# RTCartist/Neuromorphic-Spatiotemporal-Optical-Flow

Measured on AMD Instinct MI355X. Metric: 1080p frame-pairs/sec (Farneback, HIP), higher is better.
Workload: dtype f32

## Files before the change

include/nsof.h:

```cpp
#ifndef NSOF_H
#define NSOF_H

#include <stddef.h>
#include <stdint.h>

#ifdef __cplusplus
extern "C" {
#endif

#define NSOF_ABI_VERSION 3

typedef enum nsof_status {
    NSOF_OK = 0,
    NSOF_EINVAL = -1,
    NSOF_ESHAPE = -2,
    NSOF_EDEVICE = -3,
    NSOF_ENOMEM = -4,
    NSOF_EUNSUPPORTED = -5
} nsof_status;

typedef struct nsof_ctx nsof_ctx;

int nsof_create(int device, nsof_ctx** out);
void nsof_destroy(nsof_ctx* ctx);
// ... 131 lines not shown
                                       const int32_t* d_rects, int max_rects, float* d_flows, double pyr_scale, int levels,
                                       int winsize, int iterations, int poly_n, double poly_sigma, int flags,
                                       int gate_frame, long long* n_calls, long long* n_pixels);
int nsof_farneback_f32_roi_sequence_dev(nsof_ctx* ctx, int n_frames, const float* d_frames, ptrdiff_t row_stride,
                                        ptrdiff_t frame_stride, int width, int height, const int32_t* d_counts,
                                        const int32_t* d_rects, int max_rects, float* d_flows, double pyr_scale, int levels,
                                        int winsize, int iterations, int poly_n, double poly_sigma, int flags,
                                        int gate_frame, long long* n_calls, long long* n_pixels);
void* nsof_host_alloc(size_t bytes);
void nsof_host_free(void* p);

int nsof_farneback_effective_levels(int width, int height, double pyr_scale, int levels);
int nsof_farneback_level_size(int width, int height, double pyr_scale, int level,
                              int* level_width, int* level_height, int* blur_ksize, double* blur_sigma);

int nsof_stage_pyr_level_px(nsof_ctx* ctx, int pixel_type, int n_img, const void* d_src, ptrdiff_t row_stride,
                            ptrdiff_t img_stride, int width, int height, double pyr_scale, int level, float* d_out);
int nsof_stage_pyr_level(nsof_ctx* ctx, int n_img, const uint8_t* d_src, ptrdiff_t row_stride,
                         ptrdiff_t img_stride, int width, int height, double pyr_scale, int level, float* d_out);
int nsof_stage_pyr_level_f32(nsof_ctx* ctx, int n_img, const float* d_src, ptrdiff_t row_stride,
                             ptrdiff_t img_stride, int width, int height, double pyr_scale, int level, float* d_out);
int nsof_stage_polyexp(nsof_ctx* ctx, int n_img, const float* d_img, int width, int height,
                       int poly_n, double poly_sigma, float* d_R);
int nsof_stage_recip(nsof_ctx* ctx, long long n, const double* d_x, double* d_out, double* d_ieee);
int nsof_stage_update_matrices(nsof_ctx* ctx, int n_pairs, const float* d_R, const float* d_flow,
                               int width, int height, float* d_M);
int nsof_stage_blur_solve(nsof_ctx* ctx, int n_pairs, const float* d_M, int width, int height,
                          int winsize, float* d_flow);
int nsof_stage_gauss_blur_solve(nsof_ctx* ctx, int n_pairs, const float* d_M, int width, int height,
                                int winsize, float* d_flow);
int nsof_stage_iterate(nsof_ctx* ctx, int n_pairs, const float* d_R, const float* d_flow_in, int width, int height,
                       int winsize, float* d_flow_out);
int nsof_stage_iterate_upsample(nsof_ctx* ctx, int n_pairs, const float* d_R, const float* d_coarse_flow,
                                int src_w, int src_h, int width, int height, int winsize, double pyr_scale,
                                float* d_flow_out);
int nsof_stage_flow_upsample(nsof_ctx* ctx, int n_pairs, const float* d_src, int src_w, int src_h,
                             float* d_dst, int dst_w, int dst_h, double pyr_scale);

typedef enum nsof_kernel_id {
    NSOF_K_PREP = 0,
    NSOF_K_POLYEXP = 1,
    NSOF_K_UPSAMPLE = 2,
    NSOF_K_UPDMAT = 3,
    NSOF_K_BLUR = 4,
    NSOF_K_ACCUM = 5,
    NSOF_K_ITERATE = 6,
// ... 118 lines not shown
```

neuromorphic-spatiotemporal-optical-flow_amd/csrc/farneback_kernels.hip:

```cpp
#include <cstdlib>

#include <type_traits>

#include "nsof_internal.h"

#ifdef NSOF_PYR_FMA
#define NSOF_MADD(a, b, c) fmaf((a), (b), (c))
#define NSOF_PYR_NAME(n) n##_fma
#else
#define NSOF_MADD(a, b, c) ((a) * (b) + (c))
#define NSOF_PYR_NAME(n) n
#endif

namespace {

__device__ __forceinline__ int reflect101(int p, int len)
{
    if ((unsigned)p < (unsigned)len) return p;
    if (len == 1) return 0;
    do {
        if (p < 0) p = -p;
        else p = 2 * len - 2 - p;
    } while ((unsigned)p >= (unsigned)len);
    return p;
}

__device__ __forceinline__ void lin_coord_x(int d, double scale, int slen, int& s, float& a)
{
    float f = (float)((d + 0.5) * scale - 0.5);
    s = floor_f(f);
    a = f - s;
    if (s < 0) { s = 0; a = 0.f; }
    if (s >= slen - 1) { s = slen - 1; a = 0.f; }
}
__device__ __forceinline__ void lin_coord_y(int d, double scale, int& s, float& a)
{
    float f = (float)((d + 0.5) * scale - 0.5);
    s = floor_f(f);
    a = f - s;
}


template <typename T>
__device__ __forceinline__ float px(const T* p) { return (float)*p; }
template <typename T>
__device__ __forceinline__ const T* srow(const T* img, ptrdiff_t r, ptrdiff_t stride)
{
    return reinterpret_cast<const T*>(reinterpret_cast<const char*>(img) + r * stride);
}
template <typename T>
constexpr bool kU8 = std::is_same<T, uint8_t>::value;
template <typename T>
constexpr bool kInt = std::is_integral<T>::value;
template <typename T>
constexpr int kPPD = kInt<T> ? 4 / (int)sizeof(T) : 1;
template <typename T>
// ... 913 lines not shown
#pragma unroll
            for (int p = 0; p < 4; p++) st[wave][4 * lane + (p ^ ((lane >> 1) & 3))] = make_float4(o0[p], o1[p], o2[p], o3[p]);
        }
        {
            const int yo2 = y + wave;
            float4* q4 = reinterpret_cast<float4*>(Rb) + (unsigned)yo2 * (unsigned)W + (unsigned)x0;
#pragma unroll
            for (int k = 0; k < 4; k++) {
                const int px = 64 * k + lane;
                const float4 v = st[wave][(px & ~3) | ((px & 3) ^ ((px >> 3) & 3))];
                if (px < G::SW && yo2 < ye && x0 + px < W) nsof_store_stream4(reinterpret_cast<float*>(q4 + px), v.x, v.y, v.z, v.w);
            }
        }
    }
}

struct PolyFrame {
    const uint8_t* src0;
    const uint8_t* src1;
    long long row_stride, img_stride;
    int nsplit;
    float k0, k1;
};
template <int N, bool HET, bool FRAME = false, typename SRC = uint8_t>
__global__ __launch_bounds__(512, N <= 7 ? 8 : 1) void k_polyexp_rs(const float* __restrict__ img, float* __restrict__ R, int W, int H,
                                                     int seg_rows, nsof_poly_taps tp,
                                                     const nsof_het_item* __restrict__ items, PolyFrame fr = PolyFrame{})
{
    using G = PolyGeom<N>;
    size_t img_off, r_off;
    const uint8_t* sb = nullptr;
    long long srs = 0;
    if constexpr (HET) {
        const nsof_het_item& it = items[blockIdx.z >> 1];
        const size_t which = blockIdx.z & 1;
        W = it.wk;
        H = it.hk;
        if (blockIdx.x * G::SW >= W || blockIdx.y * seg_rows >= H) return;
        img_off = it.offI + which * (size_t)W * H;
        r_off = it.offR + which * 5 * (size_t)W * H;
        if constexpr (FRAME) {
            sb = it.src[which];
            srs = it.src_stride[which];
        }
    } else {
        img_off = (size_t)blockIdx.z * W * H;
        r_off = (size_t)blockIdx.z * 5 * W * H;
        if constexpr (FRAME) {
            const int z = blockIdx.z;
            sb = z < fr.nsplit ? fr.src0 + (ptrdiff_t)z * fr.img_stride : fr.src1 + (ptrdiff_t)(z - fr.nsplit) * fr.img_stride;
            srs = fr.row_stride;
// ... 19 lines not shown
        using RawPx = std::conditional_t<std::is_signed<SRC>::value, int, unsigned>;
        struct Raw3 {
            RawPx l, c, r;
        };
        auto fetch3 = [&](int srow) {
            const SRC* rp = reinterpret_cast<const SRC*>(sb + (ptrdiff_t)srow * srs);
            return Raw3{rp[xl], rp[xc], rp[xr]};
        };
        auto hval = [&](const Raw3& q) { return NSOF_MADD((float)q.l + (float)q.r, fr.k1, (float)q.c * fr.k0); };
        int rc_cur = 0;
        float hm = 0.f, h0 = 0.f, hp = 0.f, icur = 0.f;
        auto below = [&](int row) { return reflect101(clampi(row, 0, H - 1) + 1, H); };
        auto advance = [&](int row, const Raw3& under) {
            const int rc = clampi(row, 0, H - 1);
            if (rc != rc_cur) {
                hm = h0;
                h0 = hp;
                hp = hval(under);
                icur = NSOF_MADD(hm + hp, fr.k1, h0 * fr.k0);
                rc_cur = rc;
            }
            return icur;
        };
        float win[2 * N + 1];
        float pre[4];
        Raw3 praw[4];
        if constexpr (FRAME) {
            rc_cur = clampi(ys - N, 0, H - 1);
            hm = hval(fetch3(reflect101(rc_cur - 1, H)));
            h0 = hval(fetch3(rc_cur));
            hp = hval(fetch3(reflect101(rc_cur + 1, H)));
            icur = NSOF_MADD(hm + hp, fr.k1, h0 * fr.k0);
            win[0] = icur;
#pragma unroll
            for (int j = 1; j <= 2 * N; j++) win[j] = advance(ys - N + j, fetch3(below(ys - N + j)));
#pragma unroll
            for (int q = 0; q < 4; q++) pre[q] = advance(ys + 1 + N + q, fetch3(below(ys + 1 + N + q)));
        } else {
#pragma unroll
            for (int j = 0; j <= 2 * N; j++) win[j] = ld(ys - N + j);
#pragma unroll
            for (int q = 0; q < 4; q++) pre[q] = ld(ys + 1 + N + q);
        }
        for (int t = 0; t <= nsteps; t++) {
            if (t < nsteps) {
                const int y = ys + 4 * t, buf = t & 1;
// ... 6 lines not shown
#pragma unroll
                for (int q = 0; q < 4; q++) {
                    float t0 = win[N] * tp.g[0], t1 = 0.f, t2 = 0.f;
#pragma unroll
                    for (int k = 1; k <= N; k++) {
                        const float a = win[N - k], b = win[N + k];
                        float p = a + b;
                        t0 = t0 + tp.g[k] * p;
                        t2 = t2 + tp.xxg[k] * p;
                        p = b - a;
                        t1 = t1 + tp.xg[k] * p;
                    }
                    sr[buf][0][q][tid] = t0;
                    sr[buf][1][q][tid] = t1;
                    sr[buf][2][q][tid] = t2;
#pragma unroll
                    for (int j = 0; j < 2 * N; j++) win[j] = win[j + 1];
                    win[2 * N] = pre[q];
                }
#pragma unroll
                for (int q = 0; q < 4; q++) {
                    if constexpr (FRAME) pre[q] = advance(y + 5 + N + q, praw[q]);
                    else pre[q] = nxt[q];
                }
            }
            __syncthreads();
        }
        return;
    }

    char* Rb = reinterpret_cast<char*>(R + r_off);
    for (int t = 0; t <= nsteps; t++) {
        if (t >= 1) {
            const int y = ys + 4 * (t - 1), buf = (t - 1) & 1;
            const int yo = y + wave;
            const int xo = x0 + 4 * lane;
            if (4 * lane < G::SW && yo < ye && xo < W) {
                const unsigned opix = (unsigned)yo * (unsigned)W + (unsigned)xo;
                auto load_row = [&](int a, float (&v)[4 * G::NV]) {
                    const float4* p4 = reinterpret_cast<const float4*>(&sr[buf][a][wave][4 * lane]);
#pragma unroll
                    for (int i = 0; i < G::NV; i++) {
                        const float4 f = p4[i];
                        v[4 * i] = f.x; v[4 * i + 1] = f.y; v[4 * i + 2] = f.z; v[4 * i + 3] = f.w;
                    }
                };
// ... 380 lines not shown
            rb = r1;
        }
        if (live) {
            float2 o[NPL];
#pragma unroll
            for (int i = 0; i < NPL; i++) {
                const float2 t0 = hA[i], t1 = same ? hA[i] : hB[i];
                o[i].x = NSOF_MADD(t0.x, b0, t1.x * b1) * mul;
                o[i].y = NSOF_MADD(t0.y, b0, t1.y * b1) * mul;
            }
            float2* drow = D + (size_t)dy * dw + dx0;
            if (dx0 + 1 < dw && (dw & 1) == 0) {
                nsof_store_stream4(reinterpret_cast<float*>(drow), o[0].x, o[0].y, o[1].x, o[1].y);
            } else {
                drow[0] = o[0];
                if (dx0 + 1 < dw) drow[1] = o[1];
            }
        }
    }
}

template <int N, typename SRC = uint8_t>
void launch_polyexp_n(nsof_ctx* ctx, int n_img, const float* img, int W, int H, const nsof_poly_taps& taps, float* R,
                      const PolyFrame* fr = nullptr)
{
    using G = PolyGeom<N>;
    const int strips = (W + G::SW - 1) / G::SW;
    int segs = 1;
    while (segs < 64 && (long long)strips * n_img * segs < 2048 && (H / (segs * 2)) >= 64) segs *= 2;
    while (segs < 128 && (long long)strips * n_img * segs < 256 && (H / (segs * 2)) >= 16) segs *= 2;
    int seg_rows = ((H + segs - 1) / segs + 3) / 4 * 4;
    segs = (H + seg_rows - 1) / seg_rows;
    dim3 grid(strips, segs, n_img);
    if (fr)
        hipLaunchKernelGGL((k_polyexp_rs<N, false, true, SRC>), grid, dim3(512), 0, ctx->stream, img, R, W, H, seg_rows, taps, nullptr, *fr);
    else if (ctx->opt_polyexp_f32)
        hipLaunchKernelGGL((k_polyexp<N>), grid, dim3(256), 0, ctx->stream, img, R, W, H, seg_rows, taps, nullptr);
    else
        hipLaunchKernelGGL((k_polyexp_rs<N, false>), grid, dim3(512), 0, ctx->stream, img, R, W, H, seg_rows, taps, nullptr);
}

template <int N, typename SRC = uint8_t>
void launch_polyexp_het_n(nsof_ctx* ctx, int n_img, const nsof_het_item* items, const float* img, int W, int H,
                          const nsof_poly_taps& taps, float* R, const PolyFrame* fr = nullptr)
{
    using G = PolyGeom<N>;
    const int strips = (W + G::SW - 1) / G::SW;
    int segs = 1;
    while (segs < 64 && (long long)strips * n_img * segs < 2048 && (H / (segs * 2)) >= 64) segs *= 2;
    int seg_rows = ((H + segs - 1) / segs + 3) / 4 * 4;
    segs = (H + seg_rows - 1) / seg_rows;
    dim3 grid(strips, segs, n_img);
    if (fr) hipLaunchKernelGGL((k_polyexp_rs<N, true, true, SRC>), grid, dim3(512), 0, ctx->stream, img, R, W, H, seg_rows, taps, items, *fr);
    else hipLaunchKernelGGL((k_polyexp_rs<N, true>), grid, dim3(512), 0, ctx->stream, img, R, W, H, seg_rows, taps, items);
}

}

namespace {
template <typename T>
int prep_decim3_impl(nsof_ctx* ctx, int n_img, const T* src, ptrdiff_t row_stride, ptrdiff_t img_stride, int W, int H,
                     const nsof_blur_taps* taps, float* const* out)
{
    const int CWL = (W & 15) == 0 && kU8<T> ? 16 : 8;
    const int AL = kU8<T> ? CWL : 8;
    const bool ok = (W & 7) == 0 && (H & 7) == 0 && W >= 64 && H > 19 && (row_stride % AL) == 0 && (img_stride % AL) == 0 &&
                    (reinterpret_cast<uintptr_t>(src) % AL) == 0 && taps[0].ksize == 3 && taps[1].ksize == 9 &&
                    taps[2].ksize == 19 && n_img <= 65535;
    if (!ok) return NSOF_EUNSUPPORTED;
    nsof_prof_scope ps(ctx, NSOF_K_PREP);
    Decim3 d;
    for (int k = 0; k < 3; k++) {
        d.t[k] = taps[k];
        d.out[k] = out[k];
    }
    int src_rows = 96;
// ... 137 lines not shown
{
    switch (src_type) {
        case NSOF_SRC_U8: return prep_decim3_impl(ctx, n_img, static_cast<const uint8_t*>(src), row_stride, img_stride, W, H, taps, out);
        case NSOF_SRC_U16: return prep_decim3_impl(ctx, n_img, static_cast<const uint16_t*>(src), row_stride, img_stride, W, H, taps, out);
        case NSOF_SRC_S16: return prep_decim3_impl(ctx, n_img, static_cast<const int16_t*>(src), row_stride, img_stride, W, H, taps, out);
        default: return NSOF_EUNSUPPORTED;
    }
}

int NSOF_PYR_NAME(nsof_launch_prep)(nsof_ctx* ctx, int n_img, const void* src, ptrdiff_t row_stride, ptrdiff_t img_stride, int W,
                                    int H, int wk, int hk, const nsof_blur_taps& taps, float* out, int src_type)
{
    switch (src_type) {
        case NSOF_SRC_F32: return prep_impl(ctx, n_img, static_cast<const float*>(src), row_stride, img_stride, W, H, wk, hk, taps, out);
        case NSOF_SRC_U16: return prep_impl(ctx, n_img, static_cast<const uint16_t*>(src), row_stride, img_stride, W, H, wk, hk, taps, out);
        case NSOF_SRC_S16: return prep_impl(ctx, n_img, static_cast<const int16_t*>(src), row_stride, img_stride, W, H, wk, hk, taps, out);
        default: return prep_impl(ctx, n_img, static_cast<const uint8_t*>(src), row_stride, img_stride, W, H, wk, hk, taps, out);
    }
}

#ifndef NSOF_PYR_FMA
namespace {
template <typename SRC>
int polyexp_fused_impl(nsof_ctx* ctx, int n_img, const PolyFrame& fr, int W, int H, const nsof_poly_taps& taps, float* R)
{
    switch (taps.n) {
#define NSOF_PU(NN) case NN: launch_polyexp_n<NN, SRC>(ctx, n_img, nullptr, W, H, taps, R, &fr); break
        NSOF_PU(1); NSOF_PU(2); NSOF_PU(3); NSOF_PU(4); NSOF_PU(5); NSOF_PU(6); NSOF_PU(7); NSOF_PU(8); NSOF_PU(9); NSOF_PU(10);
#undef NSOF_PU
        default: return nsof_set_error(ctx, NSOF_EUNSUPPORTED, "poly_n=%d outside 1..%d", taps.n, NSOF_MAX_POLY_N);
    }
    NSOF_HIP(ctx, hipGetLastError());
    return NSOF_OK;
}
template <typename SRC>
int polyexp_het_impl(nsof_ctx* ctx, int nz, const nsof_het_item* d_items, int max_w, int max_h, const nsof_poly_taps& taps,
                     const float* I, float* R, const PolyFrame* fr)
{
    switch (taps.n) {
#define NSOF_PH(NN) case NN: launch_polyexp_het_n<NN, SRC>(ctx, nz, d_items, I, max_w, max_h, taps, R, fr); break
        NSOF_PH(1); NSOF_PH(2); NSOF_PH(3); NSOF_PH(4); NSOF_PH(5); NSOF_PH(6); NSOF_PH(7); NSOF_PH(8); NSOF_PH(9); NSOF_PH(10);
#undef NSOF_PH
        default: return nsof_set_error(ctx, NSOF_EUNSUPPORTED, "poly_n=%d outside 1..%d", taps.n, NSOF_MAX_POLY_N);
    }
    NSOF_HIP(ctx, hipGetLastError());
    return NSOF_OK;
}
}

int nsof_launch_polyexp_frames(nsof_ctx* ctx, int n_img, const void* src0, const void* src1, int nsplit, ptrdiff_t row_stride,
                           ptrdiff_t img_stride, int W, int H, const nsof_poly_taps& taps, float k0, float k1, float* R,
                           int src_type)
{
    nsof_prof_scope ps(ctx, NSOF_K_POLYEXP);
    const PolyFrame fr{static_cast<const uint8_t*>(src0), static_cast<const uint8_t*>(src1), (long long)row_stride,
                    (long long)img_stride, nsplit, k0, k1};
    switch (src_type) {
        case NSOF_SRC_U8: return polyexp_fused_impl<uint8_t>(ctx, n_img, fr, W, H, taps, R);
        case NSOF_SRC_U16: return polyexp_fused_impl<uint16_t>(ctx, n_img, fr, W, H, taps, R);
        case NSOF_SRC_S16: return polyexp_fused_impl<int16_t>(ctx, n_img, fr, W, H, taps, R);
        default: return nsof_set_error(ctx, NSOF_EINVAL, "fused level 0 takes integer frames only");
    }
}

int nsof_launch_polyexp(nsof_ctx* ctx, int n_img, const float* img, int W, int H, const nsof_poly_taps& taps, float* R)
{
    nsof_prof_scope ps(ctx, NSOF_K_POLYEXP);
    switch (taps.n) {
        case 1: launch_polyexp_n<1>(ctx, n_img, img, W, H, taps, R); break;
        case 2: launch_polyexp_n<2>(ctx, n_img, img, W, H, taps, R); break;
        case 3: launch_polyexp_n<3>(ctx, n_img, img, W, H, taps, R); break;
        case 4: launch_polyexp_n<4>(ctx, n_img, img, W, H, taps, R); break;
        case 5: launch_polyexp_n<5>(ctx, n_img, img, W, H, taps, R); break;
        case 6: launch_polyexp_n<6>(ctx, n_img, img, W, H, taps, R); break;
        case 7: launch_polyexp_n<7>(ctx, n_img, img, W, H, taps, R); break;
        case 8: launch_polyexp_n<8>(ctx, n_img, img, W, H, taps, R); break;
        case 9: launch_polyexp_n<9>(ctx, n_img, img, W, H, taps, R); break;
        case 10: launch_polyexp_n<10>(ctx, n_img, img, W, H, taps, R); break;
        default: return nsof_set_error(ctx, NSOF_EUNSUPPORTED, "poly_n=%d outside 1..%d", taps.n, NSOF_MAX_POLY_N);
    }
    NSOF_HIP(ctx, hipGetLastError());
    return NSOF_OK;
}

int nsof_launch_blur_solve(nsof_ctx* ctx, int n_pairs, const float* M, int W, int H, int winsize, float* flow)
{
    const int m = winsize / 2;
    if (m > 96) return nsof_set_error(ctx, NSOF_EUNSUPPORTED, "winsize=%d too large (max 193)", winsize);
    nsof_prof_scope ps(ctx, NSOF_K_BLUR);
    const int SW = (256 - 2 * m) & ~3;
    dim3 grid((W + SW - 1) / SW, 1, n_pairs);
    hipLaunchKernelGGL(k_blur_solve, grid, dim3(256), 0, ctx->stream, M, W, H, m, winsize, flow);
    NSOF_HIP(ctx, hipGetLastError());
    return NSOF_OK;
}

int nsof_launch_blur_solve_exact(nsof_ctx* ctx, int n_pairs, const float* M, int W, int H, int winsize, double* VT,
                                 float* flow)
{
    const int m = winsize / 2;
    nsof_prof_scope ps(ctx, NSOF_K_BLUR);
// ... 144 lines not shown
```

neuromorphic-spatiotemporal-optical-flow_amd/csrc/nsof_api.hip:

```cpp
#include <cctype>
#include <cfloat>
#include <cmath>
#include <cstdlib>
#include <algorithm>
#include <cstring>

#include <sys/syscall.h>
#include <unistd.h>

#include "nsof_internal.h"

static char g_create_err[512] = "";

int nsof_set_error(nsof_ctx* ctx, int code, const char* fmt, ...)
{
    char* dst = ctx ? ctx->err : g_create_err;
    va_list ap;
    va_start(ap, fmt);
    vsnprintf(dst, 512, fmt, ap);
    va_end(ap);
    return code;
}

int nsof_xsync_reserve(nsof_ctx* ctx, size_t carry_bytes, unsigned long long** carry, unsigned** tickets, unsigned** err)
// ... 503 lines not shown
        fast[i] = nsof_recip_normal(x[i]);
        ieee[i] = 1. / x[i];
    }
}

extern "C" int nsof_stage_recip(nsof_ctx* ctx, long long n, const double* d_x, double* d_out, double* d_ieee)
{
    if (!ctx || !d_x || !d_out || !d_ieee || n < 1) return NSOF_EINVAL;
    hipLaunchKernelGGL(k_recip_probe, dim3((unsigned)((n + 255) / 256)), dim3(256), 0, ctx->stream, n, d_x, d_out, d_ieee);
    NSOF_HIP(ctx, hipGetLastError());
    return NSOF_OK;
}

extern "C" int nsof_stage_polyexp(nsof_ctx* ctx, int n_img, const float* d_img, int width, int height, int poly_n,
                                  double poly_sigma, float* d_R)
{
    if (!ctx || !d_img || !d_R || n_img < 1 || width < 1 || height < 1) return NSOF_EINVAL;
    nsof_poly_taps taps;
    int rc = nsof_host_poly_taps(poly_n, poly_sigma, &taps);
    if (rc) return nsof_set_error(ctx, rc, "poly_n=%d unsupported", poly_n);
    return nsof_launch_polyexp(ctx, n_img, d_img, width, height, taps, d_R);
}

extern "C" int nsof_stage_update_matrices(nsof_ctx* ctx, int n_pairs, const float* d_R, const float* d_flow,
                                          int width, int height, float* d_M)
{
    if (!ctx || !d_R || !d_flow || !d_M || n_pairs < 1 || width < 1 || height < 1) return NSOF_EINVAL;
    const size_t plane = (size_t)width * height;
    return nsof_launch_update_matrices(ctx, n_pairs, d_R, d_R + 5 * plane, 10 * plane, d_flow, width, height, d_M);
}

extern "C" int nsof_stage_blur_solve(nsof_ctx* ctx, int n_pairs, const float* d_M, int width, int height,
                                     int winsize, float* d_flow)
{
    if (!ctx || !d_M || !d_flow || n_pairs < 1 || width < 1 || height < 1 || winsize < 2) return NSOF_EINVAL;
    if (nsof_form_exact(nsof_iterate_form(ctx, winsize, width, height, 1, n_pairs * nsof_iterate_jobs(width, height), 0))) {
        const size_t need = (size_t)n_pairs * 5 * width * height * sizeof(double);
        if (int rc = ctx->ws.reserve(ctx, need)) return rc;
        return nsof_launch_blur_solve_exact(ctx, n_pairs, d_M, width, height, winsize, (double*)ctx->ws.p, d_flow);
    }
    return nsof_launch_blur_solve(ctx, n_pairs, d_M, width, height, winsize, d_flow);
}

extern "C" int nsof_stage_gauss_blur_solve(nsof_ctx* ctx, int n_pairs, const float* d_M, int width, int height,
                                           int winsize, float* d_flow)
{
// ... 141 lines not shown
    auto level_I = [&](int k) { return (float*)(base + cv.offI[k]); };
    auto level_R = [&](int k) { return (float*)(base + szI + cv.offR[k]); };
    float* dS = (float*)(base + szI + szR);
    float* dM = (float*)(base + szI + szR + szS);
    double* dV = (double*)(base + szI + szR + szS + szM);
    float* fb[2] = {d_flow, dS};
    const int flips = fused ? L * (1 + iterations) + iterations : L;
    int cur = flips & 1;

    const bool prep_merged = !sequence && d_next == d_prev + (ptrdiff_t)n_pairs * pair_stride;
    auto prep_level = [&](int wk, int hk, const nsof_blur_taps& bt, float* I) -> int {
        const size_t nk = (size_t)wk * hk;
        if (sequence || prep_merged)
            return NSOF_PYR_SEL(ctx, nsof_launch_prep, (int)n_img, d_prev, row_stride, pair_stride, width, height, wk, hk, bt, I, src);
        for (int i = 0; i < 2; i++)
            if (int r = NSOF_PYR_SEL(ctx, nsof_launch_prep, n_pairs, i == 0 ? d_prev : d_next, row_stride, pair_stride, width, height,
                                     wk, hk, bt, I + (size_t)i * B * nk, src))
                return r;
        return NSOF_OK;
    };

    const bool poly_frames = src != NSOF_SRC_F32 && !ctx->opt_pyr_fma && !ctx->opt_polyexp_f32 && width >= 2 && height >= 2;
    float* Ifused[4] = {nullptr, nullptr, nullptr, nullptr};
    auto level_images = [&](int k, int wk, int hk, const nsof_blur_taps& bt) -> int {
        float* Rk = level_R(k);
        if (k >= 1 && k <= 3 && Ifused[k]) return nsof_launch_polyexp(ctx, (int)n_img, Ifused[k], wk, hk, ptaps, Rk);
        if (poly_frames && k == 0 && bt.ksize == 3 && wk == width && hk == height) {
            const bool one = sequence || prep_merged;
            return nsof_launch_polyexp_frames(ctx, (int)n_img, d_prev, one ? d_prev : d_next, one ? (int)n_img : n_pairs, row_stride,
                                          pair_stride, width, height, ptaps, bt.k[1], bt.k[2], Rk, src);
        }
        if (int r = prep_level(wk, hk, bt, level_I(k))) return r;
        return nsof_launch_polyexp(ctx, (int)n_img, level_I(k), wk, hk, ptaps, Rk);
    };

    const hipStream_t mainS = ctx->stream;
    if (lat) {
        if (!ctx->side) NSOF_HIP(ctx, hipStreamCreateWithFlags(&ctx->side, hipStreamNonBlocking));
        while (ctx->ov_events.size() < (size_t)(L + 2)) {
            hipEvent_t ev;
            NSOF_HIP(ctx, hipEventCreateWithFlags(&ev, hipEventDisableTiming));
            ctx->ov_events.push_back(ev);
        }
        struct StreamSwap {
            nsof_ctx* cx; hipStream_t saved;
            StreamSwap(nsof_ctx* cc, hipStream_t st) : cx(cc), saved(cc->stream) { cx->stream = st; }
            ~StreamSwap() { cx->stream = saved; }
        };
        const hipStream_t sideS = ctx->side;
        NSOF_HIP(ctx, hipEventRecord(ctx->ov_events[L + 1], mainS));
        NSOF_HIP(ctx, hipStreamWaitEvent(sideS, ctx->ov_events[L + 1], 0));
        for (int k = L; k >= 0; k--) {
            int wk, hk;
            nsof_blur_taps bt;
            if ((rc = nsof_level_geom(ctx, width, height, pyr_scale, k, &wk, &hk, &bt))) return rc;
            StreamSwap sw(ctx, k == L ? mainS : sideS);
            if ((rc = level_images(k, wk, hk, bt))) return rc;
// ... 15 lines not shown
            const bool one = sequence || prep_merged;
            rc = NSOF_PYR_SEL(ctx, nsof_launch_prep_decim3, one ? (int)n_img : n_pairs, d_prev, row_stride, pair_stride, width, height, bt3, I3, src);
            if (rc == NSOF_OK && !one) {
                float* I3n[3] = {I3[0] + B * nk3[0], I3[1] + B * nk3[1], I3[2] + B * nk3[2]};
                rc = NSOF_PYR_SEL(ctx, nsof_launch_prep_decim3, n_pairs, d_next, row_stride, pair_stride, width, height, bt3, I3n, src);
            }
            if (rc == NSOF_OK) {
                for (int k = 1; k <= 3; k++) Ifused[k] = I3[k - 1];
            } else if (rc != NSOF_EUNSUPPORTED) {
                return rc;
            }
        }
    }

    int pw = 0, ph = 0;
    for (int k = L; k >= 0; k--) {
        int wk, hk;
        nsof_blur_taps btaps;
        if ((rc = nsof_level_geom(ctx, width, height, pyr_scale, k, &wk, &hk, &btaps))) return rc;
        const size_t nk = (size_t)wk * hk;
        if (k == L) {
            NSOF_HIP(ctx, hipMemsetAsync(fb[cur], 0, B * nk * 8, mainS));
        } else {
            if ((rc = NSOF_PYR_SEL(ctx, nsof_launch_flow_upsample, n_pairs, fb[cur], pw, ph, fb[cur ^ 1], wk, hk,
                                   (float)(1. / pyr_scale))))
                return rc;
            cur ^= 1;
        }
        if (!lat) {
            if ((rc = level_images(k, wk, hk, btaps))) return rc;
        } else if (k < L) {
            NSOF_HIP(ctx, hipStreamWaitEvent(mainS, ctx->ov_events[k], 0));
        }
        const float* R0 = level_R(k);
        const float* R1 = R0 + (sequence ? (size_t)1 : B) * 5 * nk;
        if (fused) {
            for (int it = 0; it < iterations; it++) {
                if (form == NSOF_ITER_EXACT_LAT)
                    rc = nsof_launch_iterate_lat(ctx, n_pairs, R0, R1, 5 * nk, fb[cur], fb[cur ^ 1], wk, hk, winsize, dM, dV);
                else if (form == NSOF_ITER_EXACT)
                    rc = nsof_launch_iterate_x(ctx, n_pairs, R0, R1, 5 * nk, fb[cur], fb[cur ^ 1], wk, hk, winsize);
                else
                    rc = nsof_launch_iterate(ctx, n_pairs, R0, R1, 5 * nk, fb[cur], fb[cur ^ 1], wk, hk, winsize);
                if (rc) return rc;
                cur ^= 1;
            }
        } else {
            float* flow = fb[cur];
            for (int it = 0; it < iterations; it++) {
                if ((rc = nsof_launch_update_matrices(ctx, n_pairs, R0, R1, 5 * nk, flow, wk, hk, dM))) return rc;
                if (form == NSOF_ITER_UNFUSED_GAUSS) rc = nsof_launch_gauss_blur_solve(ctx, n_pairs, dM, wk, hk, winsize, flow);
                else if (form == NSOF_ITER_UNFUSED_EXACT) rc = nsof_launch_blur_solve_exact(ctx, n_pairs, dM, wk, hk, winsize, dV, flow);
                else rc = nsof_launch_blur_solve(ctx, n_pairs, dM, wk, hk, winsize, flow);
// ... 211 lines not shown
```

neuromorphic-spatiotemporal-optical-flow_amd/csrc/nsof_internal.h:

```cpp
#pragma once
#include <hip/hip_runtime.h>

#include <cstdarg>
#include <cstdio>
#include <utility>
#include <vector>

#include "nsof.h"

#define NSOF_MAX_POLY_N 10
#define NSOF_MAX_BLUR_TAPS 64

struct nsof_prof_slot {
    std::vector<hipEvent_t> start, stop;
    size_t used = 0;
    double acc_ms = 0;
    long long acc_launches = 0;
};

struct nsof_ctx;

int nsof_buf_grow(nsof_ctx* ctx, bool pinned, void** p, size_t* cap, size_t need, size_t new_cap);
template <class T, bool Pinned> struct nsof_buf {
    T* p = nullptr;
// ... 146 lines not shown
int nsof_launch_prep_het(nsof_ctx* ctx, int n_items, const nsof_het_item* d_items, const nsof_het_item* h_items,
                         bool level0, const nsof_blur_taps& taps, float* I, int src_type);
int nsof_launch_polyexp_het(nsof_ctx* ctx, int n_items, const nsof_het_item* d_items, int max_w, int max_h,
                            const nsof_poly_taps& taps, const float* I, float* R, const float* blur3,
                            int src_type);
int nsof_launch_flow_upsample_het(nsof_ctx* ctx, int n_items, const nsof_het_item* d_items, int max_w, int max_h,
                                  const float* src, float* dst, float mul);
int nsof_launch_iterate_het(nsof_ctx* ctx, int n_items, const nsof_het_item* d_items, int max_w, const float* R,
                            const float* flow_in, float* flow_out, bool final, int winsize);
int nsof_launch_prep(nsof_ctx* ctx, int n_img, const void* src, ptrdiff_t row_stride, ptrdiff_t img_stride, int W,
                     int H, int wk, int hk, const nsof_blur_taps& taps, float* out, int src_type);
int nsof_launch_prep_fma(nsof_ctx* ctx, int n_img, const void* src, ptrdiff_t row_stride, ptrdiff_t img_stride, int W,
                         int H, int wk, int hk, const nsof_blur_taps& taps, float* out, int src_type);
int nsof_launch_prep_decim3(nsof_ctx* ctx, int n_img, const void* src, ptrdiff_t row_stride, ptrdiff_t img_stride, int W,
                            int H, const nsof_blur_taps* taps, float* const* out, int src_type);
int nsof_launch_prep_decim3_fma(nsof_ctx* ctx, int n_img, const void* src, ptrdiff_t row_stride, ptrdiff_t img_stride,
                                int W, int H, const nsof_blur_taps* taps, float* const* out, int src_type);
int nsof_launch_prep_het_fma(nsof_ctx* ctx, int n_items, const nsof_het_item* d_items, const nsof_het_item* h_items,
                             bool level0, const nsof_blur_taps& taps, float* I, int src_type);
int nsof_launch_flow_upsample_fma(nsof_ctx* ctx, int n_pairs, const float* src, int sw, int sh, float* dst, int dw,
                                  int dh, float mul);
int nsof_launch_flow_upsample_het_fma(nsof_ctx* ctx, int n_items, const nsof_het_item* d_items, int max_w, int max_h,
                                      const float* src, float* dst, float mul);
int nsof_launch_polyexp(nsof_ctx* ctx, int n_img, const float* img, int W, int H, const nsof_poly_taps& taps,
                        float* R);
int nsof_launch_polyexp_frames(nsof_ctx* ctx, int n_img, const void* src0, const void* src1, int nsplit, ptrdiff_t row_stride,
                           ptrdiff_t img_stride, int W, int H, const nsof_poly_taps& taps, float k0, float k1, float* R,
                           int src_type);
int nsof_launch_blur_solve(nsof_ctx* ctx, int n_pairs, const float* M, int W, int H, int winsize, float* flow);
int nsof_launch_blur_solve_exact(nsof_ctx* ctx, int n_pairs, const float* M, int W, int H, int winsize, double* VT,
                                 float* flow);
#define NSOF_GAUSS_LDS_MAX_M 16
#define NSOF_GAUSS_MAX_M 96
struct nsof_gauss_taps {
    float k[NSOF_GAUSS_MAX_M + 1];
};
int nsof_launch_gauss_blur_solve(nsof_ctx* ctx, int n_pairs, const float* M, int W, int H, int winsize, float* flow);
int nsof_launch_flow_upsample(nsof_ctx* ctx, int n_pairs, const float* src, int sw, int sh, float* dst, int dw,
                              int dh, float mul);
#define NSOF_PYR_SEL(ctx, fn, ...) ((ctx)->opt_pyr_fma ? fn##_fma(ctx, __VA_ARGS__) : fn(ctx, __VA_ARGS__))
int nsof_launch_iterate(nsof_ctx* ctx, int n_pairs, const float* R0, const float* R1, size_t pair_stride,
                        const float* flow_in, float* flow_out, int W, int H, int winsize);
int nsof_launch_iterate_x(nsof_ctx* ctx, int n_pairs, const float* R0, const float* R1, size_t pair_stride,
                          const float* flow_in, float* flow_out, int W, int H, int winsize);
#define NSOF_X_STRIP 192
int nsof_launch_iterate_x_het(nsof_ctx* ctx, int n_items, const nsof_het_item* d_items, int max_w, int max_h, const float* R,
                              size_t R_floats, const float* flow_in, float* flow_out, bool final, int winsize,
                              const unsigned* d_xjobs, int stride, int njobs);

static inline bool nsof_iterate_supported(int winsize, int W, int H)
{
// ... 74 lines not shown
```

neuromorphic-spatiotemporal-optical-flow_amd/nsof/_lib.py:

```python
import ctypes as C
import importlib.util
import os


_HERE = os.path.dirname(os.path.abspath(__file__))
LIB_PATH = os.environ.get("NSOF_LIB", os.path.join(_HERE, "libnsof.so"))

OPT_POLYEXP_F32 = 1
OPT_EXACT_ROWSUMS = 2
OPT_ROW_BANDS = 3
OPT_PYR_FMA = 4
OPT_SMALL_BATCH_JOBS = 5
OPT_DEBUG_FAULT = 100
NSOF_OK, NSOF_EINVAL, NSOF_ESHAPE, NSOF_EDEVICE, NSOF_ENOMEM, NSOF_EUNSUPPORTED = 0, -1, -2, -3, -4, -5
PIXEL_U8, PIXEL_F32, PIXEL_U16, PIXEL_S16 = 0, 1, 2, 3
K_PREP, K_POLYEXP, K_UPSAMPLE, K_UPDMAT, K_BLUR, K_ACCUM, K_ITERATE, K_SEGMENT, K_MORPH, K_REMAP, K_SSIM, K_COUNT = range(12)

_vp, _i, _d, _f, _sz, _pd, _i64 = C.c_void_p, C.c_int, C.c_double, C.c_float, C.c_size_t, C.c_ssize_t, C.c_int64

class PairDesc(C.Structure):
    _fields_ = [("prev", _vp), ("prev_stride", _pd), ("next", _vp), ("next_stride", _pd), ("width", _i), ("height", _i),
                ("flow", _vp), ("flow_stride", _pd)]


# ... 14 lines not shown
    out = {}
    for name, args in _TYPED.items():
        out[name] = (_i, args)
        for infix in ("" if name.startswith("nsof_stage") else "_u8", "_f32"):
            out[name.replace("_px", infix, 1)] = (_i, args[:1] + args[2:])
    return out


SIGNATURES = {
    **_typed_signatures(),
    "nsof_create": (_i, [_i, C.POINTER(_vp)]),
    "nsof_destroy": (None, [_vp]),
    "nsof_last_error": (C.c_char_p, [_vp]),
    "nsof_abi_version": (_i, []),
    "nsof_set_stream": (_i, [_vp, _vp]),
    "nsof_synchronize": (_i, [_vp]),
    "nsof_set_option": (_i, [_vp, _i, _i]),
    "nsof_get_option": (_i, [_vp, _i, C.POINTER(_i)]),
    "nsof_host_alloc": (_vp, [_sz]),
    "nsof_host_free": (None, [_vp]),
    "nsof_farneback_effective_levels": (_i, [_i, _i, _d, _i]),
    "nsof_farneback_level_size": (_i, [_i, _i, _d, _i, C.POINTER(_i), C.POINTER(_i), C.POINTER(_i), C.POINTER(_d)]),
    "nsof_stage_polyexp": (_i, [_vp, _i, _vp, _i, _i, _i, _d, _vp]),
    "nsof_stage_recip": (_i, [_vp, C.c_longlong, _vp, _vp, _vp]),
    "nsof_stage_update_matrices": (_i, [_vp, _i, _vp, _vp, _i, _i, _vp]),
    "nsof_stage_blur_solve": (_i, [_vp, _i, _vp, _i, _i, _i, _vp]),
    "nsof_stage_gauss_blur_solve": (_i, [_vp, _i, _vp, _i, _i, _i, _vp]),
    "nsof_stage_iterate": (_i, [_vp, _i, _vp, _vp, _i, _i, _i, _vp]),
    "nsof_stage_iterate_upsample": (_i, [_vp, _i, _vp, _vp, _i, _i, _i, _i, _i, _d, _vp]),
    "nsof_stage_flow_upsample": (_i, [_vp, _i, _vp, _i, _i, _vp, _i, _i, _d]),
    "nsof_prof_enable": (_i, [_vp, C.c_uint]),
    "nsof_prof_collect": (_i, [_vp, _i, C.POINTER(_d), C.POINTER(C.c_longlong)]),
    "nsof_kernel_name": (C.c_char_p, [_i]),
    "nsof_accum_create": (_i, [_vp, _i, _i, _i, _i, _f, _f, C.POINTER(_vp)]),
    "nsof_accum_destroy": (None, [_vp]),
    "nsof_accum_set_dense": (_i, [_vp, _i]),
    "nsof_accum_reset": (_i, [_vp]),
    "nsof_accum_step_events": (_i, [_vp, _vp, _vp, _vp, _vp, _vp, _i64, _i64]),
    "nsof_accum_set_events": (_i, [_vp, _vp, _vp, _vp, _vp, _vp, _i64]),
    "nsof_accum_set_slice_times": (_i, [_vp, _vp, _vp, _i64]),
    "nsof_accum_run": (_i, [_vp, _i64, _i64, _i64]),
    "nsof_accum_surface_u8_dev": (_i, [_vp, _i, _i, _vp, _pd]),
    "nsof_accum_surface_f32_dev": (_i, [_vp, _i, _i, _vp, _pd]),
    "nsof_accum_run_surface": (_i, [_vp, _i64, _i64, _i, _i, _vp, _pd]),
    "nsof_accum_run_frames": (_i, [_vp, _i64, _i64, _i64, _i, _i, _vp, _pd, _pd]),
    "nsof_accum_set_frames_path": (_i, [_vp, _i]),
# ... 68 lines not shown
```

Measured before the change: 7110.

## Fold coarse-to-fine flow upsample into polynomial expansion kernel

```diff
diff --git a/include/nsof.h b/include/nsof.h
--- a/include/nsof.h
+++ b/include/nsof.h
@@ -177,6 +177,9 @@
                              ptrdiff_t img_stride, int width, int height, double pyr_scale, int level, float* d_out);
 int nsof_stage_polyexp(nsof_ctx* ctx, int n_img, const float* d_img, int width, int height,
                        int poly_n, double poly_sigma, float* d_R);
+int nsof_stage_polyexp_upsample(nsof_ctx* ctx, int n_img, const float* d_img, int width, int height, int poly_n,
+                                double poly_sigma, float* d_R, int n_flow, const float* d_coarse_flow, int src_w,
+                                int src_h, double pyr_scale, float* d_flow_out);
 int nsof_stage_recip(nsof_ctx* ctx, long long n, const double* d_x, double* d_out, double* d_ieee);
 int nsof_stage_update_matrices(nsof_ctx* ctx, int n_pairs, const float* d_R, const float* d_flow,
                                int width, int height, float* d_M);
diff --git a/neuromorphic-spatiotemporal-optical-flow_amd/csrc/farneback_kernels.hip b/neuromorphic-spatiotemporal-optical-flow_amd/csrc/farneback_kernels.hip
--- a/neuromorphic-spatiotemporal-optical-flow_amd/csrc/farneback_kernels.hip
+++ b/neuromorphic-spatiotemporal-optical-flow_amd/csrc/farneback_kernels.hip
@@ -25,13 +25,17 @@
     return p;
 }
 
-__device__ __forceinline__ void lin_coord_x(int d, double scale, int slen, int& s, float& a)
-{
-    float f = (float)((d + 0.5) * scale - 0.5);
+__device__ __forceinline__ float lin_coord_f(int d, double scale) { return (float)((d + 0.5) * scale - 0.5); }
+__device__ __forceinline__ void lin_split_x(float f, int slen, int& s, float& a)
+{
     s = floor_f(f);
     a = f - s;
     if (s < 0) { s = 0; a = 0.f; }
     if (s >= slen - 1) { s = slen - 1; a = 0.f; }
+}
+__device__ __forceinline__ void lin_coord_x(int d, double scale, int slen, int& s, float& a)
+{
+    lin_split_x(lin_coord_f(d, scale), slen, s, a);
 }
 __device__ __forceinline__ void lin_coord_y(int d, double scale, int& s, float& a)
 {
@@ -991,11 +995,27 @@
     int nsplit;
     float k0, k1;
 };
-template <int N, bool HET, bool FRAME = false, typename SRC = uint8_t>
+__device__ __forceinline__ float add_in_order(float a, float b)
+{
+    float r;
+    asm("v_add_f32 %0, %1, %2" : "=v"(r) : "v"(a), "v"(b));
+    return r;
+}
+#define NSOF_KEEP_IN_LOOP(v) asm volatile("" : "+v"(v))
+struct PolyUps {
+    const float* src;
+    float* dst;
+    double scale_x, scale_y;
+    int sw, sh, n_flow;
+    float mul;
+};
+template <int N, bool HET, bool FRAME = false, bool UPS = false, typename SRC = uint8_t>
 __global__ __launch_bounds__(512, N <= 7 ? 8 : 1) void k_polyexp_rs(const float* __restrict__ img, float* __restrict__ R, int W, int H,
                                                      int seg_rows, nsof_poly_taps tp,
-                                                     const nsof_het_item* __restrict__ items, PolyFrame fr = PolyFrame{})
-{
+                                                     const nsof_het_item* __restrict__ items, PolyFrame fr = PolyFrame{},
+                                                     PolyUps up = PolyUps{})
+{
+    static_assert(!(UPS && HET), "work lists keep the separate resample kernel");
     using G = PolyGeom<N>;
     size_t img_off, r_off;
     const uint8_t* sb = nullptr;
@@ -1061,6 +1081,40 @@
             }
             return icur;
         };
+        struct UpsRaw {
+            float2 p0, p1;
+        };
+        bool ups = false;
+        if constexpr (UPS) ups = (int)blockIdx.z < up.n_flow;
+        const float2* US = nullptr;
+        float2* UD = nullptr;
+        float uf = 0.f;
+        bool uown = false;
+        int usy = 0;
+        float2 hA = make_float2(0.f, 0.f), hB = hA;
+        auto ufetch = [&](int srow, unsigned uc0) {
+            const unsigned r0 = (unsigned)clampi(srow, 0, up.sh - 1) * (unsigned)up.sw;
+            const char* Sb = reinterpret_cast<const char*>(US);
+            return UpsRaw{*reinterpret_cast<const float2*>(Sb + (r0 + uc0) * 8u),
+                          *reinterpret_cast<const float2*>(Sb + (r0 + min(uc0 + 1u, (unsigned)up.sw - 1u)) * 8u)};
+        };
+        auto ublend = [&](const UpsRaw& v, float ua1) {
+            const float ua0 = 1.f - ua1;
+            return make_float2(add_in_order(v.p0.x * ua0, v.p1.x * ua1), add_in_order(v.p0.y * ua0, v.p1.y * ua1));
+        };
+        if (ups) {
+            int sx;
+            float ua1;
+            uf = lin_coord_f(xc, up.scale_x);
+            lin_split_x(uf, up.sw, sx, ua1);
+            US = reinterpret_cast<const float2*>(up.src) + (size_t)blockIdx.z * (size_t)up.sw * (size_t)up.sh;
+            UD = reinterpret_cast<float2*>(up.dst) + (size_t)blockIdx.z * plane;
+            uown = tid >= G::NP && tid < G::NP + G::SW && x0 - G::NP + tid < W;
+            float b;
+            lin_coord_y(ys, up.scale_y, usy, b);
+            hA = ublend(ufetch(usy, (unsigned)sx), ua1);
+            hB = ublend(ufetch(usy + 1, (unsigned)sx), ua1);
+        }
         float win[2 * N + 1];
         float pre[4];
         Raw3 praw[4];
@@ -1113,6 +1167,36 @@
                 for (int q = 0; q < 4; q++) {
                     if constexpr (FRAME) pre[q] = advance(y + 5 + N + q, praw[q]);
                     else pre[q] = nxt[q];
+                }
+                if (ups) {
+                    NSOF_KEEP_IN_LOOP(uf);
+                    int sx;
+                    float ua1;
+                    lin_split_x(uf, up.sw, sx, ua1);
+                    int ucol = xc, ul = tid;
+                    NSOF_KEEP_IN_LOOP(ucol);
+                    NSOF_KEEP_IN_LOOP(ul);
+                    int usq[4], ls;
+                    float ub1[4], lb;
+                    lin_coord_y(y + (ul & 3), up.scale_y, ls, lb);
+#pragma unroll
+                    for (int q = 0; q < 4; q++) {
+                        usq[q] = __builtin_amdgcn_readlane(ls, q);
+                        ub1[q] = __int_as_float(__builtin_amdgcn_readlane(__float_as_int(lb), q));
+                    }
+#pragma unroll
+                    for (int q = 0; q < 4; q++) {
+                        if (usq[q] != usy) {
+                            hA = hB;
+                            hB = ublend(ufetch(usq[q] + 1, (unsigned)sx), ua1);
+                            usy = usq[q];
+                        }
+                        if (uown && y + q < ye) {
+                            const float b1 = ub1[q], b0 = 1.f - b1;
+                            nsof_store_stream2(reinterpret_cast<float*>(reinterpret_cast<char*>(UD) + ((unsigned)(y + q) * (unsigned)W + (unsigned)ucol) * 8u),
+                                               add_in_order(hA.x * b0, hB.x * b1) * up.mul, add_in_order(hA.y * b0, hB.y * b1) * up.mul);
+                        }
+                    }
                 }
             }
             __syncthreads();
@@ -1539,7 +1623,7 @@
 
 template <int N, typename SRC = uint8_t>
 void launch_polyexp_n(nsof_ctx* ctx, int n_img, const float* img, int W, int H, const nsof_poly_taps& taps, float* R,
-                      const PolyFrame* fr = nullptr)
+                      const PolyFrame* fr = nullptr, const nsof_poly_ups* ups = nullptr)
 {
     using G = PolyGeom<N>;
     const int strips = (W + G::SW - 1) / G::SW;
@@ -1549,8 +1633,16 @@
     int seg_rows = ((H + segs - 1) / segs + 3) / 4 * 4;
     segs = (H + seg_rows - 1) / seg_rows;
     dim3 grid(strips, segs, n_img);
-    if (fr)
-        hipLaunchKernelGGL((k_polyexp_rs<N, false, true, SRC>), grid, dim3(512), 0, ctx->stream, img, R, W, H, seg_rows, taps, nullptr, *fr);
+    if (ups) {
+        const PolyUps up{ups->coarse, ups->fine, 1. / ((double)W / ups->sw), 1. / ((double)H / ups->sh), ups->sw, ups->sh,
+                         ups->n_flow, ups->mul};
+        if (fr)
+            hipLaunchKernelGGL((k_polyexp_rs<N, false, true, true, SRC>), grid, dim3(512), 0, ctx->stream, img, R, W, H, seg_rows, taps, nullptr, *fr, up);
+        else
+            hipLaunchKernelGGL((k_polyexp_rs<N, false, false, true>), grid, dim3(512), 0, ctx->stream, img, R, W, H, seg_rows, taps, nullptr,
+                               PolyFrame{}, up);
+    } else if (fr)
+        hipLaunchKernelGGL((k_polyexp_rs<N, false, true, false, SRC>), grid, dim3(512), 0, ctx->stream, img, R, W, H, seg_rows, taps, nullptr, *fr);
     else if (ctx->opt_polyexp_f32)
         hipLaunchKernelGGL((k_polyexp<N>), grid, dim3(256), 0, ctx->stream, img, R, W, H, seg_rows, taps, nullptr);
     else
@@ -1568,7 +1660,7 @@
     int seg_rows = ((H + segs - 1) / segs + 3) / 4 * 4;
     segs = (H + seg_rows - 1) / seg_rows;
     dim3 grid(strips, segs, n_img);
-    if (fr) hipLaunchKernelGGL((k_polyexp_rs<N, true, true, SRC>), grid, dim3(512), 0, ctx->stream, img, R, W, H, seg_rows, taps, items, *fr);
+    if (fr) hipLaunchKernelGGL((k_polyexp_rs<N, true, true, false, SRC>), grid, dim3(512), 0, ctx->stream, img, R, W, H, seg_rows, taps, items, *fr);
     else hipLaunchKernelGGL((k_polyexp_rs<N, true>), grid, dim3(512), 0, ctx->stream, img, R, W, H, seg_rows, taps, items);
 }
 
@@ -1752,15 +1844,25 @@
 #ifndef NSOF_PYR_FMA
 namespace {
 template <typename SRC>
-int polyexp_fused_impl(nsof_ctx* ctx, int n_img, const PolyFrame& fr, int W, int H, const nsof_poly_taps& taps, float* R)
+int polyexp_fused_impl(nsof_ctx* ctx, int n_img, const PolyFrame& fr, int W, int H, const nsof_poly_taps& taps, float* R,
+                       const nsof_poly_ups* ups)
 {
     switch (taps.n) {
-#define NSOF_PU(NN) case NN: launch_polyexp_n<NN, SRC>(ctx, n_img, nullptr, W, H, taps, R, &fr); break
+#define NSOF_PU(NN) case NN: launch_polyexp_n<NN, SRC>(ctx, n_img, nullptr, W, H, taps, R, &fr, ups); break
         NSOF_PU(1); NSOF_PU(2); NSOF_PU(3); NSOF_PU(4); NSOF_PU(5); NSOF_PU(6); NSOF_PU(7); NSOF_PU(8); NSOF_PU(9); NSOF_PU(10);
 #undef NSOF_PU
         default: return nsof_set_error(ctx, NSOF_EUNSUPPORTED, "poly_n=%d outside 1..%d", taps.n, NSOF_MAX_POLY_N);
     }
     NSOF_HIP(ctx, hipGetLastError());
+    return NSOF_OK;
+}
+int polyexp_ups_check(nsof_ctx* ctx, int n_img, int W, int H, const nsof_poly_ups* ups)
+{
+    if (!ups) return NSOF_OK;
+    if (ctx->opt_polyexp_f32) return nsof_set_error(ctx, NSOF_EUNSUPPORTED, "the float expansion carries no flow resample");
+    if (!ups->coarse || !ups->fine || ups->n_flow < 1 || ups->n_flow > n_img || ups->sw < 1 || ups->sh < 1 || ups->sw > W || ups->sh > H)
+        return nsof_set_error(ctx, NSOF_EINVAL, "flow resample %dx%d -> %dx%d of %d pairs on %d images", ups->sw, ups->sh, W, H,
+                              ups->n_flow, n_img);
     return NSOF_OK;
 }
 template <typename SRC>
@@ -1780,33 +1882,36 @@
 
 int nsof_launch_polyexp_frames(nsof_ctx* ctx, int n_img, const void* src0, const void* src1, int nsplit, ptrdiff_t row_stride,
                            ptrdiff_t img_stride, int W, int H, const nsof_poly_taps& taps, float k0, float k1, float* R,
-                           int src_type)
-{
+                           int src_type, const nsof_poly_ups* ups)
+{
+    if (int rc = polyexp_ups_check(ctx, n_img, W, H, ups)) return rc;
     nsof_prof_scope ps(ctx, NSOF_K_POLYEXP);
     const PolyFrame fr{static_cast<const uint8_t*>(src0), static_cast<const uint8_t*>(src1), (long long)row_stride,
                     (long long)img_stride, nsplit, k0, k1};
     switch (src_type) {
-        case NSOF_SRC_U8: return polyexp_fused_impl<uint8_t>(ctx, n_img, fr, W, H, taps, R);
-        case NSOF_SRC_U16: return polyexp_fused_impl<uint16_t>(ctx, n_img, fr, W, H, taps, R);
-        case NSOF_SRC_S16: return polyexp_fused_impl<int16_t>(ctx, n_img, fr, W, H, taps, R);
+        case NSOF_SRC_U8: return polyexp_fused_impl<uint8_t>(ctx, n_img, fr, W, H, taps, R, ups);
+        case NSOF_SRC_U16: return polyexp_fused_impl<uint16_t>(ctx, n_img, fr, W, H, taps, R, ups);
+        case NSOF_SRC_S16: return polyexp_fused_impl<int16_t>(ctx, n_img, fr, W, H, taps, R, ups);
         default: return nsof_set_error(ctx, NSOF_EINVAL, "fused level 0 takes integer frames only");
     }
 }
 
-int nsof_launch_polyexp(nsof_ctx* ctx, int n_img, const float* img, int W, int H, const nsof_poly_taps& taps, float* R)
-{
+int nsof_launch_polyexp(nsof_ctx* ctx, int n_img, const float* img, int W, int H, const nsof_poly_taps& taps, float* R,
+                        const nsof_poly_ups* ups)
+{
+    if (int rc = polyexp_ups_check(ctx, n_img, W, H, ups)) return rc;
     nsof_prof_scope ps(ctx, NSOF_K_POLYEXP);
     switch (taps.n) {
-        case 1: launch_polyexp_n<1>(ctx, n_img, img, W, H, taps, R); break;
-        case 2: launch_polyexp_n<2>(ctx, n_img, img, W, H, taps, R); break;
-        case 3: launch_polyexp_n<3>(ctx, n_img, img, W, H, taps, R); break;
-        case 4: launch_polyexp_n<4>(ctx, n_img, img, W, H, taps, R); break;
-        case 5: launch_polyexp_n<5>(ctx, n_img, img, W, H, taps, R); break;
-        case 6: launch_polyexp_n<6>(ctx, n_img, img, W, H, taps, R); break;
-        case 7: launch_polyexp_n<7>(ctx, n_img, img, W, H, taps, R); break;
-        case 8: launch_polyexp_n<8>(ctx, n_img, img, W, H, taps, R); break;
-        case 9: launch_polyexp_n<9>(ctx, n_img, img, W, H, taps, R); break;
-        case 10: launch_polyexp_n<10>(ctx, n_img, img, W, H, taps, R); break;
+        case 1: launch_polyexp_n<1>(ctx, n_img, img, W, H, taps, R, nullptr, ups); break;
+        case 2: launch_polyexp_n<2>(ctx, n_img, img, W, H, taps, R, nullptr, ups); break;
+        case 3: launch_polyexp_n<3>(ctx, n_img, img, W, H, taps, R, nullptr, ups); break;
+        case 4: launch_polyexp_n<4>(ctx, n_img, img, W, H, taps, R, nullptr, ups); break;
+        case 5: launch_polyexp_n<5>(ctx, n_img, img, W, H, taps, R, nullptr, ups); break;
+        case 6: launch_polyexp_n<6>(ctx, n_img, img, W, H, taps, R, nullptr, ups); break;
+        case 7: launch_polyexp_n<7>(ctx, n_img, img, W, H, taps, R, nullptr, ups); break;
+        case 8: launch_polyexp_n<8>(ctx, n_img, img, W, H, taps, R, nullptr, ups); break;
+        case 9: launch_polyexp_n<9>(ctx, n_img, img, W, H, taps, R, nullptr, ups); break;
+        case 10: launch_polyexp_n<10>(ctx, n_img, img, W, H, taps, R, nullptr, ups); break;
         default: return nsof_set_error(ctx, NSOF_EUNSUPPORTED, "poly_n=%d outside 1..%d", taps.n, NSOF_MAX_POLY_N);
     }
     NSOF_HIP(ctx, hipGetLastError());
diff --git a/neuromorphic-spatiotemporal-optical-flow_amd/csrc/nsof_api.hip b/neuromorphic-spatiotemporal-optical-flow_amd/csrc/nsof_api.hip
--- a/neuromorphic-spatiotemporal-optical-flow_amd/csrc/nsof_api.hip
+++ b/neuromorphic-spatiotemporal-optical-flow_amd/csrc/nsof_api.hip
@@ -549,6 +549,19 @@
     return nsof_launch_polyexp(ctx, n_img, d_img, width, height, taps, d_R);
 }
 
+extern "C" int nsof_stage_polyexp_upsample(nsof_ctx* ctx, int n_img, const float* d_img, int width, int height, int poly_n,
+                                           double poly_sigma, float* d_R, int n_flow, const float* d_coarse_flow, int src_w,
+                                           int src_h, double pyr_scale, float* d_flow_out)
+{
+    if (!ctx || !d_img || !d_R || !d_coarse_flow || !d_flow_out || n_img < 1 || width < 1 || height < 1) return NSOF_EINVAL;
+    if (ctx->opt_pyr_fma) return nsof_set_error(ctx, NSOF_EUNSUPPORTED, "NSOF_OPT_PYR_FMA keeps the separate flow resample");
+    nsof_poly_taps taps;
+    int rc = nsof_host_poly_taps(poly_n, poly_sigma, &taps);
+    if (rc) return nsof_set_error(ctx, rc, "poly_n=%d unsupported", poly_n);
+    const nsof_poly_ups ups{d_coarse_flow, d_flow_out, src_w, src_h, n_flow, (float)(1. / pyr_scale)};
+    return nsof_launch_polyexp(ctx, n_img, d_img, width, height, taps, d_R, &ups);
+}
+
 extern "C" int nsof_stage_update_matrices(nsof_ctx* ctx, int n_pairs, const float* d_R, const float* d_flow,
                                           int width, int height, float* d_M)
 {
@@ -736,17 +749,18 @@
 
     const bool poly_frames = src != NSOF_SRC_F32 && !ctx->opt_pyr_fma && !ctx->opt_polyexp_f32 && width >= 2 && height >= 2;
     float* Ifused[4] = {nullptr, nullptr, nullptr, nullptr};
-    auto level_images = [&](int k, int wk, int hk, const nsof_blur_taps& bt) -> int {
+    auto level_images = [&](int k, int wk, int hk, const nsof_blur_taps& bt, const nsof_poly_ups* ups = nullptr) -> int {
         float* Rk = level_R(k);
-        if (k >= 1 && k <= 3 && Ifused[k]) return nsof_launch_polyexp(ctx, (int)n_img, Ifused[k], wk, hk, ptaps, Rk);
+        if (k >= 1 && k <= 3 && Ifused[k]) return nsof_launch_polyexp(ctx, (int)n_img, Ifused[k], wk, hk, ptaps, Rk, ups);
         if (poly_frames && k == 0 && bt.ksize == 3 && wk == width && hk == height) {
             const bool one = sequence || prep_merged;
             return nsof_launch_polyexp_frames(ctx, (int)n_img, d_prev, one ? d_prev : d_next, one ? (int)n_img : n_pairs, row_stride,
-                                          pair_stride, width, height, ptaps, bt.k[1], bt.k[2], Rk, src);
+                                          pair_stride, width, height, ptaps, bt.k[1], bt.k[2], Rk, src, ups);
         }
         if (int r = prep_level(wk, hk, bt, level_I(k))) return r;
-        return nsof_launch_polyexp(ctx, (int)n_img, level_I(k), wk, hk, ptaps, Rk);
+        return nsof_launch_polyexp(ctx, (int)n_img, level_I(k), wk, hk, ptaps, Rk, ups);
     };
+    const bool ups_fold = !lat && !ctx->opt_polyexp_f32 && !ctx->opt_pyr_fma;
 
     const hipStream_t mainS = ctx->stream;
     if (lat) {
@@ -808,13 +822,19 @@
         if (k == L) {
             NSOF_HIP(ctx, hipMemsetAsync(fb[cur], 0, B * nk * 8, mainS));
         } else {
-            if ((rc = NSOF_PYR_SEL(ctx, nsof_launch_flow_upsample, n_pairs, fb[cur], pw, ph, fb[cur ^ 1], wk, hk,
-                                   (float)(1. / pyr_scale))))
-                return rc;
+            if (ups_fold) {
+                const nsof_poly_ups ups{fb[cur], fb[cur ^ 1], pw, ph, n_pairs, (float)(1. / pyr_scale)};
+                rc = level_images(k, wk, hk, btaps, &ups);
+            } else {
+                rc = NSOF_PYR_SEL(ctx, nsof_launch_flow_upsample, n_pairs, fb[cur], pw, ph, fb[cur ^ 1], wk, hk,
+                                  (float)(1. / pyr_scale));
+            }
+            if (rc) return rc;
             cur ^= 1;
         }
         if (!lat) {
-            if ((rc = level_images(k, wk, hk, btaps))) return rc;
+            if (k == L || !ups_fold)
+                if ((rc = level_images(k, wk, hk, btaps))) return rc;
         } else if (k < L) {
             NSOF_HIP(ctx, hipStreamWaitEvent(mainS, ctx->ov_events[k], 0));
         }
diff --git a/neuromorphic-spatiotemporal-optical-flow_amd/csrc/nsof_internal.h b/neuromorphic-spatiotemporal-optical-flow_amd/csrc/nsof_internal.h
--- a/neuromorphic-spatiotemporal-optical-flow_amd/csrc/nsof_internal.h
+++ b/neuromorphic-spatiotemporal-optical-flow_amd/csrc/nsof_internal.h
@@ -192,11 +192,17 @@
                                   int dh, float mul);
 int nsof_launch_flow_upsample_het_fma(nsof_ctx* ctx, int n_items, const nsof_het_item* d_items, int max_w, int max_h,
                                       const float* src, float* dst, float mul);
+struct nsof_poly_ups {
+    const float* coarse;
+    float* fine;
+    int sw, sh, n_flow;
+    float mul;
+};
 int nsof_launch_polyexp(nsof_ctx* ctx, int n_img, const float* img, int W, int H, const nsof_poly_taps& taps,
-                        float* R);
+                        float* R, const nsof_poly_ups* ups = nullptr);
 int nsof_launch_polyexp_frames(nsof_ctx* ctx, int n_img, const void* src0, const void* src1, int nsplit, ptrdiff_t row_stride,
                            ptrdiff_t img_stride, int W, int H, const nsof_poly_taps& taps, float k0, float k1, float* R,
-                           int src_type);
+                           int src_type, const nsof_poly_ups* ups = nullptr);
 int nsof_launch_blur_solve(nsof_ctx* ctx, int n_pairs, const float* M, int W, int H, int winsize, float* flow);
 int nsof_launch_blur_solve_exact(nsof_ctx* ctx, int n_pairs, const float* M, int W, int H, int winsize, double* VT,
                                  float* flow);
diff --git a/neuromorphic-spatiotemporal-optical-flow_amd/nsof/_lib.py b/neuromorphic-spatiotemporal-optical-flow_amd/nsof/_lib.py
--- a/neuromorphic-spatiotemporal-optical-flow_amd/nsof/_lib.py
+++ b/neuromorphic-spatiotemporal-optical-flow_amd/nsof/_lib.py
@@ -60,6 +60,7 @@
     "nsof_farneback_effective_levels": (_i, [_i, _i, _d, _i]),
     "nsof_farneback_level_size": (_i, [_i, _i, _d, _i, C.POINTER(_i), C.POINTER(_i), C.POINTER(_i), C.POINTER(_d)]),
     "nsof_stage_polyexp": (_i, [_vp, _i, _vp, _i, _i, _i, _d, _vp]),
+    "nsof_stage_polyexp_upsample": (_i, [_vp, _i, _vp, _i, _i, _i, _d, _vp, _i, _vp, _i, _i, _d, _vp]),
     "nsof_stage_recip": (_i, [_vp, C.c_longlong, _vp, _vp, _vp]),
     "nsof_stage_update_matrices": (_i, [_vp, _i, _vp, _vp, _i, _i, _vp]),
     "nsof_stage_blur_solve": (_i, [_vp, _i, _vp, _i, _i, _i, _vp]),
```

Result: no change. 7163 (median of 6 runs) (+0.7%).
